# jonathan-laurent/AlphaZero.jl

Measured on AMD Instinct MI355X. Metric: self-play MCTS sims/sec (Connect-Four, 4096 parallel games per GPU), higher is better.
Workload: dtype f32

## Files before the change

### alphazero.jl_amd/csrc/azhip.hip

```cpp
#include "engine.h"
#include "minmax.h"

static thread_local std::string g_err;
int fail(int code, const char* fmt, ...) {
  char buf[512];
  va_list ap;
  va_start(ap, fmt);
  vsnprintf(buf, sizeof buf, fmt, ap);
  va_end(ap);
  g_err = buf;
  return code;
}
extern "C" const char* az_last_error(void) { return g_err.c_str(); }
extern "C" int az_debug_scratch_live_bytes(int64_t* bytes) {
  if (!bytes) return fail(AZ_ERR_BAD_ARG, "NULL argument");
  *bytes = (int64_t)scratch_live_bytes.load();
  return AZ_OK;
}
extern "C" int az_abi_version(void) { return AZ_ABI_VERSION; }
extern "C" int az_abi_struct_size(int32_t which) {
  switch (which) {
    case AZ_STRUCT_ENGINE_CFG: return (int)sizeof(az_engine_cfg);
    case AZ_STRUCT_MOVE_REC: return (int)sizeof(az_move_rec);
    case AZ_STRUCT_GAME_REC: return (int)sizeof(az_game_rec);
// ... 277 lines not shown
    long long plies = c->game == AZ_GAME_MANCALA ? 128 : gi.max_plies;
    cap = (long long)c->num_iters_per_turn * plies * std::max(1, c->reset_every);
    if (c->reset_every == 0) cap *= 4;
    cap = std::max<long long>(cap, 1024);
  }
  if (cap > (1LL << 30)) return fail(AZ_ERR_BAD_ARG, "max_nodes_per_slot too large");
  v.cap_nodes = (int)cap;
  int hs = 1024;
  while ((long long)hs * 2 < cap * 3) hs <<= 1;
  v.ht_size = hs;
  v.tag_mask = e->env.tag_mask; v.epoch0 = e->env.epoch0; v.bk_mode = e->env.bk_mode;
  AZCHK(dalloc(e, &v.sr, G)); AZCHK(dalloc(e, &v.game_id, G));
  AZCHK(dalloc(e, &v.move_idx, G)); AZCHK(dalloc(e, &e->d_node_count, G));
  AZCHK(dalloc(e, &v.worker_sim_id, G));
  AZCHK(dalloc(e, &v.eta, (size_t)G * gi.APAD));
  AZCHK(dalloc(e, &v.ht, (size_t)G * hs));
  AZCHK(create_node_pool(e));
  AZCHK(dalloc(e, &v.path, (size_t)G * v.max_depth));
  AZCHK(dalloc(e, &v.leaf_env, G));
  AZCHK(dalloc(e, &v.eval_slots, (size_t)2 * G)); v.eval_stride = G;
  AZCHK(dalloc(e, &v.bg_list, (size_t)2 * G)); AZCHK(dalloc(e, &v.bg_cnt, 2 * AZ_MAX_GROUPS));
  return dalloc(e, &v.n_eval, 2 * AZ_MAX_GROUPS);
}

static int create_side_records(az_engine* e) {
  DView& v = e->v; const int G = v.G;
  const size_t piece = (size_t)e->vm_chunk_nodes * 32;
  void* kbase = nullptr;
  bool mapped_keys = e->vm_rows > 0 && e->env.vmm_keys && piece > 0 && VM_CHUNK % piece == 0;
  size_t kbytes = 0;
  if (mapped_keys) {
    kbytes = ((size_t)e->vm_rows * G * piece + VM_CHUNK - 1) / VM_CHUNK * VM_CHUNK;
    if (hipMemAddressReserve(&kbase, kbytes, VM_CHUNK, nullptr, 0) != hipSuccess) { (void)hipGetLastError(); mapped_keys = false; }
  }
  if (mapped_keys) {
    e->vmk_base = (char*)kbase; e->vmk_bytes = kbytes; e->vmk_piece = piece;
    e->vmk_granule.assign(kbytes / VM_CHUNK, 0);
    v.keys = (unsigned long long*)kbase;
    v.key_row = (size_t)G * piece / 8; v.key_stride = piece / 8;
  } else {
    AZCHK(dalloc(e, &v.keys, (size_t)G * v.cap_nodes * 4, false));
    v.key_row = 0; v.key_stride = (size_t)v.cap_nodes * 4;
    if (e->vm_rows) v.key_row = (size_t)e->vm_chunk_nodes * 4;
  }
  hipLaunchKernelGGL(k_slot_records, dim3((G + 255) / 256), dim3(256), 0, e->stream, v, (int)SR_ZERO);
  return AZ_OK;
}

static int create_eval_cache(az_engine* e) {
  const az_engine_cfg* c = &e->cfg; const GameInfo& gi = e->gi; DView& v = e->v; const int G = v.G;
  AZCHK(dalloc(e, &v.Pout, (size_t)std::max(G, 1) * gi.APAD)); AZCHK(dalloc(e, &v.Vout, G));
  const bool on = e->env.eval_cache >= 0 ? e->env.eval_cache != 0 && c->oracle != AZ_ORACLE_ROLLOUT : oracle_is_net(*c);
  if (!on || e->env.use_graphs) return AZ_OK;
  int lg = e->env.eval_cache_log2;
  if (!lg) for (lg = 16; lg < 24 && ((long long)1 << lg) < 8LL * G * std::max(1, c->num_iters_per_turn);) ++lg;
  AZCHK(dalloc(e, &e->d_ec, (size_t)1 << lg));
  e->ec_mask = ((uint32_t)1 << lg) - 1u;
  AZCHK(dalloc(e, &e->d_ec_claim, (size_t)2 * G, false));
  HIPCHK(hipMemsetAsync(e->d_ec_claim, 0xff, sizeof(int) * 2 * (size_t)G, e->stream));
  AZCHK(dalloc(e, &e->d_Phit, (size_t)G * gi.APAD)); AZCHK(dalloc(e, &e->d_Vhit, G));
  v.ec = e->d_ec; v.ec_mask = e->ec_mask; v.ec_seq = 0; v.ec_claim = e->d_ec_claim; v.Phit = e->d_Phit; v.Vhit = e->d_Vhit;
  return AZ_OK;
}

static constexpr size_t FETCH_BYTES = (size_t)1 << 20;
static int create_words(az_engine* e) {
  DView& v = e->v; const int G = v.G;
  AZCHK(dalloc(e, &v.trace, (size_t)G * v.max_moves)); AZCHK(dalloc(e, &v.grec, G));
  AZCHK(dalloc(e, &v.finished, G)); AZCHK(dalloc(e, &v.err, 1));
  AZCHK(dalloc(e, &e->d_xerr, AZ_MAX_GROUPS + 1)); AZCHK(dalloc(e, &e->d_skipped, 2 * (AZ_MAX_GROUPS + 1)));
  v.xerr = e->d_xerr + AZ_MAX_GROUPS; v.skipped = e->d_skipped + 2 * AZ_MAX_GROUPS;
  AZCHK(halloc_mapped(e, &e->h_xflag, &e->d_xflag, 1, 0));
  AZCHK(halloc_mapped(e, &e->h_nleaf, &e->d_nleaf, AZ_MAX_GROUPS, -1));
  AZCHK(halloc_mapped(e, &e->h_needy, &e->d_needy, AZ_MAX_GROUPS, 0));
  AZCHK(dalloc(e, &e->d_fr, 1)); AZCHK(dalloc(e, &e->d_bg_stop, 1));
  AZCHK(halloc_mapped(e, &e->h_busy, &e->d_busy, AZ_MAX_GROUPS, -1));
  AZCHK(halloc_pinned(e, &e->h_report, 1, hipHostMallocMapped));
  memset(e->h_report, 0, sizeof *e->h_report);
  HIPCHK(hipHostGetDevicePointer((void**)&e->d_report, e->h_report, 0));
  AZCHK(halloc_pinned(e, &e->h_fetch, FETCH_BYTES));
  return halloc_mapped(e, &e->h_fr_words, &e->d_fr_words, 2, 0);
}

static int create_staging(az_engine* e) {
  const int G = e->v.G;
  e->io_cap = std::max(G, 4096);
  AZCHK(dalloc(e, &e->d_slots, e->io_cap)); AZCHK(dalloc(e, &e->d_gids, e->io_cap)); AZCHK(dalloc(e, &e->d_roots, e->io_cap));
  AZCHK(dalloc(e, &e->d_moves, e->io_cap)); AZCHK(dalloc(e, &e->d_eta, (size_t)e->io_cap * AZ_MAX_ACTIONS));
  AZCHK(dalloc(e, &e->d_offsets, e->io_cap)); AZCHK(dalloc(e, &e->d_stage, (size_t)G * e->v.max_moves));
  AZCHK(dalloc(e, &e->d_keys, (size_t)2 * e->io_cap)); AZCHK(dalloc(e, &e->d_actions, e->io_cap));
  AZCHK(dalloc(e, &e->d_next, (size_t)2 * e->io_cap)); AZCHK(dalloc(e, &e->d_term, e->io_cap)); AZCHK(dalloc(e, &e->d_reward, e->io_cap));
  AZCHK(dalloc(e, &e->d_nodebuf, 512));
  return dalloc(e, &e->d_visits, (size_t)e->io_cap * (AZ_MAX_ACTIONS + 1));
}

static int create_net_buffers(az_engine* e) {
  const az_engine_cfg* c = &e->cfg; const GameInfo& gi = e->gi;
  e->nn_cap = e->io_cap;
  if (c->oracle != AZ_ORACLE_SIMPLENET) AZCHK(dalloc(e, &e->d_hfeat, (size_t)e->nn_cap * gi.P * std::max(64, c->num_filters), false));
  AZCHK(dalloc(e, &e->d_X, (size_t)e->nn_cap * gi.C * gi.P)); AZCHK(dalloc(e, &e->d_A, (size_t)e->nn_cap * gi.A));
  AZCHK(dalloc(e, &e->d_P, (size_t)e->nn_cap * std::max(16, gi.APAD))); AZCHK(dalloc(e, &e->d_V, e->nn_cap)); AZCHK(dalloc(e, &e->d_Pinv, e->nn_cap));
  AZCHK(dalloc(e, &e->d_tmp_env, e->nn_cap)); AZCHK(dalloc(e, &e->d_iota, e->nn_cap)); AZCHK(dalloc(e, &e->d_ntmp, 1));
  AZCHK(halloc_pinned(e, &e->h_env, (size_t)e->nn_cap)); AZCHK(halloc_pinned(e, &e->h_n, 1)); AZCHK(halloc_pinned(e, &e->h_pv, (size_t)e->nn_cap * (gi.A + 1)));
  hipLaunchKernelGGL(k_iota, dim3((e->nn_cap + 255) / 256), dim3(256), 0, e->stream, e->d_iota, e->nn_cap);
  e->xch_epoch = e->env.xch_epoch0;
  { hipDeviceProp_t pr; HIPCHK(hipGetDeviceProperties(&pr, c->device)); e->num_cu = pr.multiProcessorCount; }
  return net_set_kernel_attrs(e);
}

static int create_groups(az_engine* e) {
  const az_engine_cfg* c = &e->cfg; const GameInfo& gi = e->gi; DView& v = e->v; const int G = v.G;
  if (e->env.tree_sort) { AZCHK(dalloc(e, &e->d_perm, (size_t)2 * G)); AZCHK(dalloc(e, &e->d_perm_prev, (size_t)2 * G)); }
  int ng = std::min(std::max(c->batch_size > 0 ? G / c->batch_size : 1, 1), (int)AZ_MAX_GROUPS);
  while (ng > 1 && G % ng != 0) --ng;
// ... 391 lines not shown
    HIPCHK(hipStreamSynchronize(e->stream));
  }
  HIPCHK(hipGetLastError());
  if (e->xch_epoch) AZCHK(check_device_error(e));
  return AZ_OK;
}

static int evaluate_envs(az_engine* e, const std::vector<GEnv>& envs, std::vector<float>& P, std::vector<float>& V) {
  const GameInfo& gi = e->gi;
  const int N = (int)envs.size();
  P.assign((size_t)N * gi.A, 0.f); V.assign(N, 0.f);
  for (int off = 0; off < N; off += e->nn_cap) {
    int m = std::min(e->nn_cap, N - off);
    HIPCHK(hipMemcpyAsync(e->d_tmp_env, envs.data() + off, sizeof(GEnv) * m, hipMemcpyHostToDevice, e->stream));
    HIPCHK(hipMemcpyAsync(e->d_ntmp, &m, sizeof(int), hipMemcpyHostToDevice, e->stream));
    AZCHK(seam_launch(e, false, m));
    HIPCHK(hipMemcpyAsync(P.data() + (size_t)gi.A * off, e->d_P, sizeof(float) * gi.A * m, hipMemcpyDeviceToHost, e->stream));
    HIPCHK(hipMemcpyAsync(V.data() + off, e->d_V, sizeof(float) * m, hipMemcpyDeviceToHost, e->stream));
    HIPCHK(hipStreamSynchronize(e->stream));
  }
  HIPCHK(hipGetLastError());
  if (e->xch_epoch) AZCHK(check_device_error(e));
  return AZ_OK;
}

extern "C" int az_net_evaluate_keys(az_engine* e, const uint64_t* keys, int32_t N, float* P, float* V) {
  ENGINE(e);
  if (!e->net_loaded) return fail(AZ_ERR_STATE, "az_net_set_params has not been called");
  if (N < 0 || (N > 0 && (!keys || !P || !V))) return fail(AZ_ERR_BAD_ARG, "NULL buffer");
  const GameInfo& gi = e->gi;
  for (int off = 0; off < N; off += e->nn_cap) {
    const int m = std::min(e->nn_cap, N - off);
    GEnv* envs = e->h_env;
    DISPATCH_GAME(e->cfg.game, { for (int i = 0; i < m; ++i) envs[i] = Gm::from_key(keys[2 * (size_t)(off + i)], keys[2 * (size_t)(off + i) + 1]); });
    *e->h_n = m;
    float* hP = e->h_pv; float* hV = e->h_pv + (size_t)gi.A * e->nn_cap;
    HIPCHK(hipMemcpyAsync(e->d_tmp_env, envs, sizeof(GEnv) * m, hipMemcpyHostToDevice, e->stream));
    HIPCHK(hipMemcpyAsync(e->d_ntmp, e->h_n, sizeof(int), hipMemcpyHostToDevice, e->stream));
    AZCHK(seam_launch(e, false, m));
    HIPCHK(hipMemcpyAsync(hP, e->d_P, sizeof(float) * gi.A * m, hipMemcpyDeviceToHost, e->stream));
    HIPCHK(hipMemcpyAsync(hV, e->d_V, sizeof(float) * m, hipMemcpyDeviceToHost, e->stream));
    HIPCHK(hipStreamSynchronize(e->stream));
    memcpy(P + (size_t)gi.A * off, hP, sizeof(float) * gi.A * m);
    memcpy(V + off, hV, sizeof(float) * m);
  }
  HIPCHK(hipGetLastError());
  if (e->xch_epoch) AZCHK(check_device_error(e));
  return AZ_OK;
}

static int ec_empty(az_engine* e, bool wipe) {
  if (!e->d_ec) return AZ_OK;
  AZCHK(sync_all(e));
  if (wipe) HIPCHK(hipMemsetAsync(e->d_ec, 0, sizeof(ECEnt) * ((size_t)e->ec_mask + 1), e->stream));
  HIPCHK(hipMemsetAsync(e->d_ec_claim, 0xff, sizeof(int) * 2 * (size_t)e->v.G, e->stream));
  HIPCHK(hipStreamSynchronize(e->stream));
  if (wipe) e->ec_seq = 0;
  e->v.ec_floor = e->ec_seq;
  for (int g = 0; g < e->ngroups; ++g) e->gv[g].ec_floor = e->ec_seq;
  return AZ_OK;
}
static int ec_next_launch(az_engine* e, DView* v) {
  if (!e->d_ec) return AZ_OK;
  if (e->ec_seq >= (1u << 29)) AZCHK(ec_empty(e, true));
  v->ec_seq = ++e->ec_seq;
  return AZ_OK;
}
template <class Gm> static int wave_group(az_engine* e, int g, uint32_t sim_idx) {
  constexpr int L = Gm::APAD;
  AZCHK(ec_next_launch(e, &e->gv[g]));
  const DView& v = e->gv[g];
  hipStream_t st = e->gs[g], sn = e->gt[g];
  const bool split = st != sn;
  const int G = v.G;
  const int gb = (G * L + 255) / 256;
  const int par = (e->wave_par[g] ^= 1);
  e->ph.stats.slot_launches += e->group_active[g];
  LAUNCH_ON(e, st, AZ_K_SELECT, G, (k_tree<Gm>), gb, 256, 0, v, e->p, (e->pending[g] || e->ph.fr_on) ? 1 : 0, 1, par);
  e->pending[g] = true;
  hipStream_t s2 = st;
  e->bg_signal = false;
  const bool side = e->ph.fr_on && !split && oracle_is_net(e->cfg) && e->fr_s[1] && st == e->fr_s[0];
  if (side) { s2 = e->fr_s[1]; HIPCHK(hipEventRecord(e->fr_ev[0], st)); ++e->bg_seq; e->bg_signal = env_process().bg_stop && e->ph.fr_kbg > 0; }
  if (oracle_is_net(e->cfg)) {
    AZCHK(net_wave(e, g, split, e->group_active[g]));
  } else {
    LAUNCH_ON(e, st, AZ_K_SYNTH, G, (k_synth_oracle<Gm>), (G + 255) / 256, 256, 0, v, e->p, sim_idx, par);
  }
  if (e->ph.fr_on) {
    FRArgs fa;
    fa.st = e->d_fr; fa.done = e->d_done; fa.done_off = e->d_done_off;
    fa.recs = e->d_phase ? e->d_phase : e->d_stage; fa.recs_cap = e->d_phase ? (long long)e->phase_cap : (long long)e->v.G * e->v.max_moves;
    fa.done_cap = e->done_cap; fa.total_games = e->ph.ids.total_games; fa.first_game_id = (uint32_t)e->ph.ids.first_game_id; fa.group = g; fa.host_words = e->d_fr_words;
    hipStream_t s3 = side ? e->fr_s[2] : s2;
    if (side) { HIPCHK(hipStreamWaitEvent(s2, e->fr_ev[0], 0)); HIPCHK(hipStreamWaitEvent(s3, e->fr_ev[0], 0)); }
    { DView mv = v; mv.low_prio = env_process().bg_prio ? 0 : 1; LAUNCH_ON(e, s3, AZ_K_MOVE, G, (k_move_fr<Gm>), (G + 255) / 256, 256, 0, mv, e->p, fa); }
    if (e->ph.fr_kbg > 0) {
      AZCHK(ec_next_launch(e, &e->gv[g]));
      DView bv = e->gv[g];
      bv.run_k = e->ph.fr_kbg; bv.low_prio = env_process().bg_prio ? 0 : 1;
      if (side && e->bg_signal) { bv.bg_stop = e->d_bg_stop; bv.bg_seq = e->bg_seq; }
      LAUNCH_ON(e, s2, AZ_K_EXPAND, G, (k_tree<Gm>), gb, 256, 0, bv, e->p, 0, 1, par ^ 1);
    }
    if (side) {
      HIPCHK(hipEventRecord(e->fr_ev[2], s3)); HIPCHK(hipStreamWaitEvent(s2, e->fr_ev[2], 0));
      HIPCHK(hipEventRecord(e->fr_ev[1], s2)); HIPCHK(hipStreamWaitEvent(st, e->fr_ev[1], 0));
    }
// ... 929 lines not shown
```

### alphazero.jl_amd/csrc/engine.h

```cpp
#pragma once
#include <hip/hip_runtime.h>

#include <algorithm>
#include <atomic>
#include <chrono>
#include <cmath>
#include <cstdarg>
#include <cstdio>
#include <cstring>
#include <new>
#include <string>
#include <map>
#include <memory>
#include <mutex>
#include <vector>
#include <unordered_set>

#include "../../include/az_numerics.h"
#include "../../include/azhip.h"
#include "env.h"
#include "games.h"
#include "net_layout.h"
#include "phase_books.h"
#include "resnet.h"
// ... 53 lines not shown
  return SimpleLayout(SimpleShape{gi.C * gi.P, gi.A, h.width, h.depth_common, h.depth_phead, h.depth_vhead, h.use_batch_norm});
}
inline bool oracle_is_net(const az_engine_cfg& c) { return c.oracle == AZ_ORACLE_RESNET || c.oracle == AZ_ORACLE_SIMPLENET; }

struct Phase {
  bool running = false;
  bool fr_on = false;
  bool host_moves = true;
  GameIds ids;
  int games_done = 0, wave_in_move = 0, active_slots = 0;
  int fr_k = 0, fr_kbg = 0, fr_round_waves = 0;
  int fr_prev_done = 0, fr_since_round = 0, fr_given_up = 0; long long fr_prev_recs = 0;
  int fr_look_waves = 0, fr_since_look = 0;
  std::vector<az_game_rec> q_games;
  std::vector<az_move_rec> q_moves;
  std::vector<az_game_rec> dev_games;
  std::vector<int64_t> dev_off; int64_t dev_n = 0;
  std::vector<int32_t> aborted_ids;
  az_selfplay_stats stats = {};
  std::chrono::steady_clock::time_point t_begin;
};
struct ProfRec { hipEvent_t a = nullptr, b = nullptr; int cls = 0; };
struct az_engine {
  az_engine_cfg cfg = {};
  az_simplenet_hp shp = {};
  GameInfo gi = {};
  EnvCreate env;
  int device = 0;
  hipStream_t stream = nullptr;
  DView v = {};
  DParams p = {};
  int ngroups = 0;
  DView gv[AZ_MAX_GROUPS] = {};
  hipStream_t gs[AZ_MAX_GROUPS] = {};
  hipStream_t gt[AZ_MAX_GROUPS] = {};
  hipEvent_t ev_tree[AZ_MAX_GROUPS] = {}, ev_net[AZ_MAX_GROUPS] = {};
  float* g_hfeat[AZ_MAX_GROUPS] = {};
  unsigned long long* xch[AZ_MAX_GROUPS + 1] = {}; unsigned long long xch_epoch = 0;
  int* d_xerr = nullptr; int* d_skipped = nullptr;
  int* h_needy = nullptr; int* d_needy = nullptr;
  int* h_nleaf = nullptr; int* d_nleaf = nullptr;
  int* h_xflag = nullptr; int* d_xflag = nullptr;
  bool split_off = false;
  long long xch_launches = 0;
  int split_registered = 0;
  std::vector<void*> allocs;
  size_t alloc_bytes = 0;
  std::vector<void*> host_allocs;
  char* vm_base = nullptr; size_t vm_bytes = 0, vm_chunk = 0; int vm_rows = 0, vm_chunk_nodes = 0;
  std::vector<hipMemGenericAllocationHandle_t> vm_handles; std::vector<char*> vm_at;
  std::vector<int> h_slot_cap, h_node_count; int* d_slot_cap = nullptr; int* d_node_count = nullptr; size_t vm_budget = 0, vm_mapped = 0;
  char* vmk_base = nullptr; size_t vmk_bytes = 0, vmk_piece = 0; std::vector<uint8_t> vmk_granule;
  int* d_perm = nullptr; long long* d_perm_prev = nullptr;
  ECEnt* d_ec = nullptr; uint32_t ec_mask = 0; uint32_t ec_seq = 0; int* d_ec_claim = nullptr; float* d_Phit = nullptr; float* d_Vhit = nullptr;
  size_t stat_words = 0; std::vector<long long> h_stat;
  std::vector<void*> net_allocs;
  bool net_loaded = false;
  std::vector<float> blob;
  std::unique_ptr<const NetMaps> net_maps;
  std::vector<unsigned char> trainable;
  NetDev net = {};
  std::unique_ptr<const SimpleMaps> simple_maps;
  SimpleDev snet = {};
  Net16bDev net16b = {};
  Net16Dev net16 = {};
  uint16_t* d_geo[GEO_COUNT] = {};
  long long tower_hist[4] = {};
  char last_tower[96] = {};
  int num_cu = 0;
  int nn_cap = 0;
  float* d_hfeat = nullptr; float* d_X = nullptr; float* d_A = nullptr; float* d_P = nullptr; float* d_V = nullptr; float* d_Pinv = nullptr;
  GEnv* d_tmp_env = nullptr; int* d_iota = nullptr; int* d_ntmp = nullptr;
  GEnv* h_env = nullptr; int* h_n = nullptr; float* h_pv = nullptr;
  int* d_slots = nullptr; uint32_t* d_gids = nullptr; GEnv* d_roots = nullptr; uint32_t* d_moves = nullptr; double* d_eta = nullptr; int* d_offsets = nullptr;
  az_move_rec* d_stage = nullptr; unsigned long long* d_keys = nullptr; int* d_actions = nullptr; unsigned long long* d_next = nullptr; signed char* d_term = nullptr; float* d_reward = nullptr;
  char* d_nodebuf = nullptr;
  int* d_visits = nullptr;
  int io_cap = 0;
  Phase ph;
  std::map<int, hipGraphExec_t> wave_graphs;
  bool pending[AZ_MAX_GROUPS] = {};
  int wave_par[AZ_MAX_GROUPS] = {};
  int group_active[AZ_MAX_GROUPS] = {};
  hipStream_t fr_s[4] = {}; hipEvent_t fr_ev[4] = {};
  FRState* d_fr = nullptr; az_game_rec* d_done = nullptr; long long* d_done_off = nullptr; int done_cap = 0;
  int* h_busy = nullptr; int* d_busy = nullptr;
  int* d_bg_stop = nullptr; int bg_seq = 0; bool bg_signal = false;
  int* h_fr_words = nullptr; int* d_fr_words = nullptr;
  std::vector<az_game_rec> h_done; std::vector<long long> h_done_off;
  StepReport* h_report = nullptr; StepReport* d_report = nullptr; bool report_fresh = false;
  char* h_fetch = nullptr;
  az_move_rec* d_phase = nullptr; int64_t phase_cap = 0;
  bool prof_on = false;
  int prof_mask = 0;
  std::vector<ProfRec> prof_pool;
  size_t prof_used = 0;
  az_prof prof = {};
  double next_exec = 1.0;
  std::vector<int> h_finished;
  std::vector<az_game_rec> h_grec;
  bool mm_on = false;
  az_minmax_cfg mm = {};
  GEnv* d_mm_roots = nullptr; double* d_mm_q = nullptr; int mm_cap = 0;
  unsigned long long* d_sv_keys = nullptr; int8_t* d_sv_q = nullptr; long long* d_sv_nodes = nullptr; int sv_cap = 0;
};

template <class T> inline int dalloc(az_engine* e, T** p, size_t n, bool zero = true) {
// ... 217 lines not shown
```

### alphazero.jl_amd/csrc/tree.h

```cpp
#pragma once
#include <hip/hip_runtime.h>
#include <stdint.h>
#include <type_traits>
#include "../../include/az_numerics.h"
#include "../../include/azhip.h"
#include "games.h"

enum { LEAF_NONE = 0, LEAF_NEW = 1, LEAF_TERMINAL = 2 };
enum { DERR_NODE_POOL = 1, DERR_HASH_FULL = 2, DERR_DEPTH = 3, DERR_MOVES = 4, DERR_NO_ROOT = 5 };

struct DParams {
  double gamma, cpuct, eps, alpha, prior_temp;
  int nsims, temp_len;
  int temp_xs[AZ_SCHED_MAX];
  double temp_ys[AZ_SCHED_MAX];
  uint64_t seed;
  int oracle, reset_every;
  double flip_p;
  int retire;
};

enum { SR_ACTIVE = 1, SR_MS_SHIFT = 8 };
struct alignas(64) SlotRec {
  unsigned long long root_a, root_b;
  long long tot_sims, tot_trav;
  uint32_t root_fin;
  int leaf_kd;
  int eidx, node_count;
  uint32_t epoch, leaf_ins;
  int root_idx, active;
  __host__ __device__ inline GEnv root() const { GEnv g; g.a = root_a; g.b = root_b; g.fin = root_fin; return g; }
  __host__ __device__ inline void set_root(const GEnv& g) { root_a = g.a; root_b = g.b; root_fin = g.fin; }
};
static_assert(sizeof(SlotRec) == 64, "slot record");

struct alignas(64) ECEnt { unsigned long long ka, kb; float P[AZ_MAX_ACTIONS]; float V; uint32_t cs; uint32_t meta; };
static_assert(sizeof(ECEnt) == 64, "evaluation cache entry");
enum { EC_EMPTY = 0, EC_PENDING = 1, EC_READY = 2, EC_FILLING = 3, EC_STALE_AFTER = 64 };

struct DView {
  int G, cap_nodes, ht_size, max_depth, max_moves;
  ECEnt* ec;
  uint32_t ec_mask, ec_seq;
  uint32_t ec_floor;
  int* ec_claim;
  int* needy_host;
  int* nleaf_host;
  float* Phit; float* Vhit;
  uint32_t tag_mask;
  uint32_t epoch0;
  SlotRec* sr;
  uint32_t* game_id;
  uint32_t* move_idx;
  int* worker_sim_id;
  double* eta;
  unsigned long long* ht;
  char* nodes;
  int node_sh; uint32_t node_mask; size_t node_row, node_stride;
  const int* slot_cap;
  unsigned long long* keys;
  size_t key_row, key_stride;
  const int* perm;
  int bk_mode;
  unsigned long long* path;
  GEnv* leaf_env;
  int* eval_slots;
  int eval_stride;
  const int* bg_stop; int bg_seq;
  int* bg_list; int* bg_cnt;
  int* n_eval;
  float* Pout;
  float* Vout;
  az_move_rec* trace;
  az_game_rec* grec;
  int* finished;
  int* err;
  int* xerr;
  int* skipped;
  long long* stat;
  unsigned long long* dbg;
  int run_k;
  int fr;
  int* busy_host;
  int low_prio;
  int slot0;
  int* fr_active;
};

static constexpr int AZ_MAX_GROUPS = 4;
struct FRState {
  unsigned long long resv;
  long long moves;
  int next_game;
  int active[AZ_MAX_GROUPS];
};
struct FRArgs {
// ... 45 lines not shown
  static_assert(L == 8 || L == 16, "lane groups of 8 or 16");
  x += dpp_partner<0>(x);
  x += dpp_partner<1>(x);
  x += dpp_partner<2>(x);
  if constexpr (L == 16) x += dpp_partner<3>(x);
  return x;
}
template <int CTRL> __device__ __forceinline__ double dpp_ctrl(double x) {
  const int lo = __builtin_amdgcn_update_dpp(0, __double2loint(x), CTRL, 0xF, 0xF, false);
  const int hi = __builtin_amdgcn_update_dpp(0, __double2hiint(x), CTRL, 0xF, 0xF, false);
  return __hiloint2double(hi, lo);
}
template <int L> __device__ __forceinline__ int group_argmax(double s, int lane, int* carry) {
  static_assert(L == 8 || L == 16, "lane groups of 8 or 16");
  constexpr int Q1 = 0xB1, Q2 = 0x4E, HM = 0x141, RM = 0x140;
  double m = __builtin_fmax(s, dpp_ctrl<Q1>(s));
  m = __builtin_fmax(m, dpp_ctrl<Q2>(m));
  m = __builtin_fmax(m, dpp_ctrl<HM>(m));
  if constexpr (L == 16) m = __builtin_fmax(m, dpp_ctrl<RM>(m));
  const unsigned long long eq = __ballot(s == m);
  const int base = (threadIdx.x & 63) & ~(L - 1);
  const int idx = __ffs((unsigned)((eq >> base) & ((1u << L) - 1u))) - 1;
  int c = (lane == idx) ? *carry : 0;
  c |= __builtin_amdgcn_update_dpp(0, c, Q1, 0xF, 0xF, false);
  c |= __builtin_amdgcn_update_dpp(0, c, Q2, 0xF, 0xF, false);
  c |= __builtin_amdgcn_update_dpp(0, c, HM, 0xF, 0xF, false);
  if constexpr (L == 16) c |= __builtin_amdgcn_update_dpp(0, c, RM, 0xF, 0xF, false);
  *carry = c;
  return idx;
}
template <int L> __device__ __forceinline__ int group_argmax(double s, int lane) { int c = 0; return group_argmax<L>(s, lane, &c); }

template <int L> __device__ __forceinline__ uint32_t group_xor(uint32_t x) {
  x ^= (uint32_t)dpp_partner<0>((int)x);
  x ^= (uint32_t)dpp_partner<1>((int)x);
  x ^= (uint32_t)dpp_partner<2>((int)x);
  if constexpr (L == 16) x ^= (uint32_t)dpp_partner<3>((int)x);
  return x;
}
template <int L> __device__ __forceinline__ int group_bcast0(int x, int lane) { return group_sum<L>(lane == 0 ? x : 0); }
__device__ __forceinline__ uint32_t ec_ld32(const uint32_t* p) { return __hip_atomic_load(p, __ATOMIC_RELAXED, __HIP_MEMORY_SCOPE_AGENT); }
__device__ __forceinline__ unsigned long long ec_ld64(const unsigned long long* p) { return __hip_atomic_load(p, __ATOMIC_RELAXED, __HIP_MEMORY_SCOPE_AGENT); }
__device__ __forceinline__ float ec_ldf(const float* p) { return __uint_as_float(__hip_atomic_load((const uint32_t*)p, __ATOMIC_RELAXED, __HIP_MEMORY_SCOPE_AGENT)); }
__device__ __forceinline__ void ec_st32(uint32_t* p, uint32_t v) { __hip_atomic_store(p, v, __ATOMIC_RELAXED, __HIP_MEMORY_SCOPE_AGENT); }
__device__ __forceinline__ void ec_st64(unsigned long long* p, unsigned long long v) { __hip_atomic_store(p, v, __ATOMIC_RELAXED, __HIP_MEMORY_SCOPE_AGENT); }
__device__ __forceinline__ void ec_stf(float* p, float v) { __hip_atomic_store((uint32_t*)p, __float_as_uint(v), __ATOMIC_RELAXED, __HIP_MEMORY_SCOPE_AGENT); }
__device__ __forceinline__ bool ec_cas(uint32_t* p, uint32_t expect, uint32_t want) {
  return __hip_atomic_compare_exchange_strong(p, &expect, want, __ATOMIC_RELAXED, __ATOMIC_RELAXED, __HIP_MEMORY_SCOPE_AGENT);
}
__device__ __forceinline__ uint32_t ec_term(float p, int lane) {
  const uint32_t b = __float_as_uint(p), r = (uint32_t)(5 * lane + 1) & 31u;
  return (b << r) | (b >> ((32u - r) & 31u));
}
__device__ __forceinline__ uint32_t ec_checksum(uint32_t px, unsigned long long ka, unsigned long long kb, float V, uint32_t ready_meta) {
  unsigned long long h = az_hash_key(ka, kb);
  h = az_mix64(h ^ (((unsigned long long)px << 32) | (unsigned long long)__float_as_uint(V)));
  h = az_mix64(h + (unsigned long long)ready_meta);
  return (uint32_t)(h >> 32) ^ (uint32_t)h;
}
__device__ __forceinline__ uint32_t ec_index(unsigned long long ka, unsigned long long kb, uint32_t mask) {
  return (uint32_t)(az_hash_key(ka, kb) >> 17) & mask;
}

template <class Gm>
__device__ inline int ht_lookup(const DView& v, int slot, int lane, unsigned long long ka,
                                unsigned long long kb, uint32_t epoch, uint32_t* ins) {
  constexpr int L = Gm::APAD;
  const unsigned long long hk = az_hash_key(ka, kb);
  const uint32_t H1 = (uint32_t)v.ht_size - 1;
  const uint32_t h0 = (uint32_t)hk & H1;
  const uint32_t tag = (uint32_t)(hk >> 40) & v.tag_mask;
  const unsigned long long* tab = v.ht + (size_t)slot * v.ht_size;
  const int iters = v.ht_size / L;
  for (int i = 0; i < iters; ++i) {
    uint32_t pos = (h0 + (uint32_t)(i * L + lane)) & H1;
    unsigned long long e = tab[pos];
    uint32_t idx1 = (uint32_t)e;
    bool live = ((uint32_t)(e >> 48) == epoch) && idx1 != 0;
    bool match = false;
    if (live && ((uint32_t)(e >> 32) & 0xffff) == tag) {
      const unsigned long long* k = side_at(v, slot, (int)(idx1 - 1));
      match = (k[0] == ka) && (k[1] == kb);
    }
    unsigned mb = group_ballot<L>(match), db = group_ballot<L>(!live);
    int fm = mb ? __ffs(mb) - 1 : 99, fd = db ? __ffs(db) - 1 : 99;
    if (fm < fd) {
      int base = (threadIdx.x & 63) & ~(L - 1);
      return (int)__shfl((int)idx1, base + fm) - 1;
    }
    if (fd != 99) { *ins = (h0 + (uint32_t)(i * L + fd)) & H1; return -1; }
  }
  dev_fail(v, DERR_HASH_FULL);
  *ins = 0;
  return -1;
}

template <class Gm>
__device__ inline void arm_noise(const DView& v, const DParams& p, int slot, const GEnv& env) {
  constexpr int L = Gm::APAD;
  uint32_t m = Gm::mask(env);
  int n = __popc(m);
  double eta[AZ_MAX_ACTIONS];
  az_rng r = az_rng_make(p.seed, v.game_id[slot], v.move_idx[slot], AZ_RNG_NOISE);
  az_dirichlet(&r, n, p.alpha, eta);
  int k = 0;
  for (int a = 0; a < L; ++a) {
    double e = 0.0;
    if (a < Gm::A && ((m >> a) & 1)) e = eta[k++];
    v.eta[(size_t)slot * L + a] = e;
  }
}

template <class Gm> __device__ inline void set_link(char* nd, int act, uint32_t link) {
  using NL = NodeL<Gm>;
  ((uint16_t*)(nd + NL::OFF_LO))[act] = (uint16_t)(link & 0xffff);
// ... 29 lines not shown
  unsigned long long st = (v.path + (size_t)slot_in * v.max_depth)[lane < v.max_depth ? lane : 0];
  GEnv lenv = v.leaf_env[slot_in];
  int kind = s0.leaf_kd & 3, depth = (s0.leaf_kd >> 2) & 0x0fffffff, e0 = s0.eidx, nc = s0.node_count;
  GEnv root0 = s0.root();
  uint32_t epoch0 = s0.epoch, ins = s0.leaf_ins;
  int ridx = s0.root_idx, active0 = s0.active;
  int claim0 = -1; uint32_t cmeta0 = 0;
  if (v.ec) { const int2 c2 = ((const int2*)v.ec_claim)[slot_in]; claim0 = c2.x; cmeta0 = (uint32_t)c2.y; }
#define AZ_PIN(x) asm volatile("" : "+v"(x))
  AZ_PIN(kind); AZ_PIN(depth); AZ_PIN(e0); AZ_PIN(nc); AZ_PIN(st); AZ_PIN(root0.a); AZ_PIN(root0.b); AZ_PIN(root0.fin);
  AZ_PIN(epoch0); AZ_PIN(ins); AZ_PIN(claim0); AZ_PIN(cmeta0); AZ_PIN(lenv.a); AZ_PIN(lenv.b); AZ_PIN(lenv.fin); AZ_PIN(ridx); AZ_PIN(active0);
  const bool mine = live && !(v.fr && kind != LEAF_NONE && (!do_backup || ((s0.leaf_kd >> 30) & 1) == par));
  if (!(do_backup && mine)) kind = LEAF_NONE;
  const int nc_in = nc, ridx_in = ridx;
  const bool inrec = lane < Gm::A;
  float Pans = 0.f, Vans = 0.f;
  if (kind == LEAF_NEW) {
    Pans = e0 >= 0 ? v.Pout[(size_t)e0 * L + lane] : v.Phit[(size_t)slot_in * L + lane];
    Vans = e0 >= 0 ? v.Vout[e0] : v.Vhit[slot_in];
  }
  const bool searching = mine && (active0 & SR_ACTIVE);
  int msims = active0 >> SR_MS_SHIFT;
  int done_sims = 0, done_trav = 0;
  int n_sel = 0, n_trav = 0, n_evl = 0, n_hit = 0;
  bool retired = false, ishit = false;
  int claim = -1; uint32_t cmeta = 0;

  for (int it = 0;; ++it) {
    KArgs ka;
    {
      auto kp = __builtin_amdgcn_kernarg_segment_ptr();
      asm volatile("" : "+s"(kp));
      __builtin_memcpy(&ka, (const void*)kp, sizeof(KArgs));
    }
    const DView& v = ka.v;
    const DParams& p = ka.p;
    int slot = slot_in; asm volatile("" : "+v"(slot));
    unsigned long long* const path = v.path + (size_t)slot * v.max_depth;
    if (kind != LEAF_NONE) {
      double q = 0.0;
      bool ok = true;
      if (kind == LEAF_NEW) {
        const int idx = nc;
        if (it == 0 && v.ec && claim0 >= 0) {
          ECEnt* const ent = v.ec + claim0;
          const float Praw = inrec ? Pans : 0.f;
          const uint32_t fill = (cmeta0 & ~3u) | EC_FILLING, ready = (cmeta0 & ~3u) | EC_READY;
          int got = 0;
          if (lane == 0) got = ec_cas(&ent->meta, cmeta0, fill) ? 1 : 0;
          got = group_bcast0<L>(got, lane);
          const uint32_t px = group_xor<L>(inrec ? ec_term(Praw, lane) : 0u);
          if (got) {
            if (inrec) ec_stf(&ent->P[lane], Praw);
            if (lane == 0) { ec_stf(&ent->V, Vans); ec_st32(&ent->cs, ec_checksum(px, lenv.a, lenv.b, Vans, ready)); }
            __builtin_amdgcn_s_waitcnt(0);
            if (lane == 0) ec_st32(&ent->meta, ready);
          }
        }
        if (idx >= (v.slot_cap ? v.slot_cap[slot] : v.cap_nodes)) {
          ok = false;
          if (!p.retire) dev_fail(v, DERR_NODE_POOL);
          else {
            retired = true;
            if (lane == 0) { v.finished[slot] = 2; if (v.fr_active) atomicSub(v.fr_active, 1); }
          }
        } else {
          const uint32_t m = Gm::mask(lenv);
          float Pf = Pans;
          if (p.prior_temp != 1.0) {
            const bool av = (m >> lane) & 1;
            double res;
            if (p.prior_temp == 0.0) {
              int am = group_argmax<L>(av ? (double)Pf : -__builtin_inf(), lane);
              res = (lane == am) ? 1.0 : 0.0;
            } else {
              double pw = av ? az_pow((double)Pf, 1.0 / p.prior_temp) : 0.0;
              double sm = 0.0;
              for (int a = 0; a < Gm::A; ++a) { double t = __shfl(pw, gbase + a); if ((m >> a) & 1) sm += t; }
              res = pw / sm;
            }
            Pf = av ? (float)res : 0.f;
          }
          if (depth == 0) ridx = idx;
          char* nd = node_at<Gm>(v, slot, idx);
          const unsigned long long st_par = (depth >= 1 && depth <= L) ? __shfl(st, gbase + depth - 1) : (depth > L ? path[depth - 1] : 0ULL);
          if (lane < Gm::A) {
            *NL::stat(nd, lane) = typename NL::Stat{0.0, 0, Pf};
            ((uint16_t*)(nd + NL::OFF_LO))[lane] = 0;
          }
          if (lane == 0) {
            *(typename NL::hi_t*)(nd + NL::OFF_HI) = 0;
            unsigned long long* kk = side_at(v, slot, idx);
            kk[0] = lenv.a; kk[1] = lenv.b; kk[2] = (unsigned long long)__float_as_uint(Vans);
            const unsigned long long hk = az_hash_key(lenv.a, lenv.b);
            const unsigned long long tag = (hk >> 40) & v.tag_mask;
            v.ht[(size_t)slot * v.ht_size + ins] =
                ((unsigned long long)epoch0 << 48) | (tag << 32) | (unsigned long long)(idx + 1);
            if (depth != 0 && links_ok)
              set_link<Gm>(node_at<Gm>(v, slot, (int)(uint32_t)st_par), (int)((st_par >> 32) & 0xff), (uint32_t)(idx + 1));
          }
          nc = idx + 1;
          q = (double)Vans;
        }
      }
      if (ok) {
        for (int c = (depth - 1) / L; c >= 0 && depth > 0; --c) {
          const int k0 = c * L, kn = (depth - k0) < L ? (depth - k0) : L;
// ... 52 lines not shown
          else if (lane == 0 && links_ok) set_link<Gm>(node_at<Gm>(v, slot, pidx), pact, (uint32_t)(idx + 1));
          have = false;
        }
        if (depth >= v.max_depth) { dev_fail(v, DERR_DEPTH); kind = LEAF_NONE; break; }
        if (!have) {
          const char* nd = node_at<Gm>(v, slot, idx);
          if (inrec) { sa = *NL::stat(nd, lane); lo = ((const uint16_t*)(nd + NL::OFF_LO))[lane]; }
          hi = *(const typename NL::hi_t*)(nd + NL::OFF_HI);
        }
        const uint32_t amask = Gm::mask(env);
        const int N = sa.N;
        const float Pf = sa.P;
        const double W = sa.W;
        const int link = (int)(lo | (((hi >> (2 * lane)) & 3u) << 16));
        if (dbg && it == 0 && depth == 0) dbg[2] = __builtin_readcyclecounter() + (unsigned long long)(N & 0);
        const int Ntot = group_sum<L>(N);
        const double sqrtNtot = __builtin_sqrt((double)Ntot);
        const double Q = W / (double)(N > 1 ? N : 1);
        double Pd = (double)Pf;
        if (depth == 0 && p.eps != 0.0) Pd = (1.0 - p.eps) * Pd + p.eps * v.eta[(size_t)slot * L + lane];
        double sc = Q + p.cpuct * Pd * sqrtNtot / (double)(N + 1);
        if (!((amask >> lane) & 1)) sc = -__builtin_inf();
        int nxt = link;
        if (dbg && it == 0 && depth == 0) dbg[7] = __builtin_readcyclecounter() + (unsigned long long)(__double2loint(sc) & 0);
        const int act = group_argmax<L>(sc, lane, &nxt);
        if (dbg && it == 0 && depth == 0) dbg[8] = __builtin_readcyclecounter() + (unsigned long long)(act & 0);
        have = nxt != 0;
        if (have) {
          const char* nd = node_at<Gm>(v, slot, nxt - 1);
          if (inrec) { sa = *NL::stat(nd, lane); lo = ((const uint16_t*)(nd + NL::OFF_LO))[lane]; }
          hi = *(const typename NL::hi_t*)(nd + NL::OFF_HI);
        }
        const bool wp = Gm::white_playing(env);
        Gm::play(env, act);
        const float wr = Gm::white_reward(env);
        const int r = (int)(wp ? wr : -wr);
        const bool psw = wp != Gm::white_playing(env);
        const unsigned long long ent = (unsigned long long)(uint32_t)idx | ((unsigned long long)act << 32) |
                                       ((unsigned long long)(psw ? 1 : 0) << 40) | ((unsigned long long)(r + 1) << 41);
        if (lane == 0) path[depth] = ent;
        if (lane == depth) st = ent;
        pidx = idx; pact = act;
        if (dbg && it == 0 && depth == 0) dbg[9] = __builtin_readcyclecounter() + (env.a & 0);
        depth++;
        probe = nxt == 0;
        idx = nxt - 1;
      }
      if (dbg && it == 0) dbg[3] = __builtin_readcyclecounter();
      lenv = env;
      if (kind != LEAF_NONE) { n_sel += 1; n_trav += depth; }
      if (kind == LEAF_NEW) {
        n_evl += 1;
        if (v.ec) {
          const uint32_t ci = ec_index(env.a, env.b, v.ec_mask);
          ECEnt* const ent = v.ec + ci;
          const uint32_t m1 = ec_ld32(&ent->meta);
          const unsigned long long ka = ec_ld64(&ent->ka), kb = ec_ld64(&ent->kb);
          const float pl = inrec ? ec_ldf(&ent->P[lane]) : 0.f;
          const float vv = ec_ldf(&ent->V);
          const uint32_t cs = ec_ld32(&ent->cs);
          const uint32_t px = group_xor<L>(inrec ? ec_term(pl, lane) : 0u);
          const bool okc = (m1 & 3u) == EC_READY && (m1 >> 2) > v.ec_floor && ka == env.a && kb == env.b && cs == ec_checksum(px, ka, kb, vv, m1);
          ishit = group_bcast0<L>(okc ? 1 : 0, lane) != 0;
          if (ishit) { Pans = inrec ? pl : 0.f; Vans = vv; n_hit += 1; }
          else {
            claim = -1; cmeta = 0;
            if (lane == 0) {
              const int32_t age = (int32_t)(v.ec_seq - (m1 >> 2));
              if (m1 == 0u || (m1 & 3u) == EC_READY || age > (int32_t)EC_STALE_AFTER || (m1 >> 2) <= v.ec_floor) {
                const uint32_t mine = (v.ec_seq << 2) | EC_PENDING;
                if (ec_cas(&ent->meta, m1, mine)) { ec_st64(&ent->ka, env.a); ec_st64(&ent->kb, env.b); claim = (int)ci; cmeta = mine; }
              }
            }
          }
        }
      }
    }
    if (kind == LEAF_NONE) break;
    if (kind == LEAF_NEW && !ishit) break;
    if (!v.run_k) break;
    __threadfence_block();
  }

  const int slot = slot_in;
  SlotRec* const sr = v.sr + slot;
  if (mine && lane == 0) {
    sr->leaf_kd = kind == LEAF_NONE ? (int)LEAF_NONE : (kind | (depth << 2) | (par << 30));
    if (do_select && kind != LEAF_NONE) { v.leaf_env[slot] = lenv; sr->leaf_ins = ins; }
    if (nc != nc_in) sr->node_count = nc;
    if (ridx != ridx_in) sr->root_idx = ridx;
    if (done_sims) { sr->tot_trav += done_trav; sr->tot_sims += done_sims; }
    const int aw = retired ? 0 : ((active0 & ((1 << SR_MS_SHIFT) - 1)) | (msims << SR_MS_SHIFT));
    if (aw != active0) sr->active = aw;
  }
  if (!do_select) return;
  if (ishit && kind == LEAF_NEW) {
    v.Phit[(size_t)slot * L + lane] = Pans;
    if (lane == 0) { v.Vhit[slot] = Vans; sr->eidx = -1; }
  }
  if (dbg) dbg[4] = __builtin_readcyclecounter();

  const bool head = mine && lane == 0;
  const bool isnew = head && kind == LEAF_NEW && !ishit;
  const unsigned long long bal = __ballot(isnew);
  const bool needy = head && v.run_k && v.bg_list && (v.fr ? (do_backup && searching && !retired && kind == LEAF_NONE && msims < p_arg.nsims)
                                                           : (kind != LEAF_NONE || (searching && !retired && msims < p_arg.nsims)));
  const unsigned long long baln = __ballot(needy);
  int sims = head ? n_sel : 0, trav = head ? n_trav : 0, evl = head ? n_evl : 0, hits = head ? n_hit : 0;
#pragma unroll
  for (int o = 32; o > 0; o >>= 1) { sims += __shfl_down(sims, o); trav += __shfl_down(trav, o); evl += __shfl_down(evl, o); hits += __shfl_down(hits, o); }
  if (wl == 0) { s_need[w] = __popcll(baln); s_new[w] = __popcll(bal); s_hit[w] = hits; s_evl[w] = evl; s_sims[w] = sims; s_trav[w] = trav; }
  __syncthreads();
  if (threadIdx.x == 0) {
    const int nw = blockDim.x >> 6;
    int tot = 0, toth = 0, te = 0, ts = 0, tt = 0;
    for (int i = 0; i < nw; ++i) { tot += s_new[i]; toth += s_hit[i]; te += s_evl[i]; ts += s_sims[i]; tt += s_trav[i]; }
    s_base = tot ? atomicAdd(v.n_eval + par, tot) : 0;
    { int tn = 0; for (int i = 0; i < nw; ++i) tn += s_need[i]; s_nbase = tn ? atomicAdd(v.bg_cnt + par, tn) : 0; }
    if (ts) {
      long long* sp = v.stat + (size_t)blockIdx.x * 4;
      sp[0] += ts; sp[1] += tt; sp[2] += te; sp[3] += toth;
    }
    if (blockIdx.x == 0 && (do_backup || !v.fr)) {
      if (v.nleaf_host && do_select) __hip_atomic_store(v.nleaf_host, v.n_eval[par ^ 1], __ATOMIC_RELAXED, __HIP_MEMORY_SCOPE_SYSTEM);
// ... 430 lines not shown
```

Measured before the change: 8.974 million.

## Make eval cache two-way set-associative and size it from free device memory

Turns the direct-mapped evaluation cache into a 2-way set-associative cache. A lookup probes both ways of a set, and a victim-selection rule prefers free, then stale, then older answered entries, and avoids evicting fresh pending claims. The default table size can now grow past 2^24 toward 2^27 entries, up to 64x the number of simulations, capped at one eighth of free device memory. The goal is a higher hit rate so fewer leaves need network evaluation, at the cost of an extra entry load per probe, more memory, and a larger wipe.

```diff
diff --git a/alphazero.jl_amd/csrc/azhip.hip b/alphazero.jl_amd/csrc/azhip.hip
--- a/alphazero.jl_amd/csrc/azhip.hip
+++ b/alphazero.jl_amd/csrc/azhip.hip
@@ -353,14 +353,15 @@
   AZCHK(dalloc(e, &v.Pout, (size_t)std::max(G, 1) * gi.APAD)); AZCHK(dalloc(e, &v.Vout, G));
   const bool on = e->env.eval_cache >= 0 ? e->env.eval_cache != 0 && c->oracle != AZ_ORACLE_ROLLOUT : oracle_is_net(*c);
   if (!on || e->env.use_graphs) return AZ_OK;
-  int lg = e->env.eval_cache_log2;
-  if (!lg) for (lg = 16; lg < 24 && ((long long)1 << lg) < 8LL * G * std::max(1, c->num_iters_per_turn);) ++lg;
-  AZCHK(dalloc(e, &e->d_ec, (size_t)1 << lg));
-  e->ec_mask = ((uint32_t)1 << lg) - 1u;
+  size_t free_b = 0, total_b = 0;
+  HIPCHK(hipMemGetInfo(&free_b, &total_b));
+  const int lg = ec_size_log2(G, c->num_iters_per_turn, e->env.eval_cache_log2, (unsigned long long)free_b);
+  e->ec_entries = (size_t)1 << lg;
+  AZCHK(dalloc(e, &e->d_ec, e->ec_entries));
   AZCHK(dalloc(e, &e->d_ec_claim, (size_t)2 * G, false));
   HIPCHK(hipMemsetAsync(e->d_ec_claim, 0xff, sizeof(int) * 2 * (size_t)G, e->stream));
   AZCHK(dalloc(e, &e->d_Phit, (size_t)G * gi.APAD)); AZCHK(dalloc(e, &e->d_Vhit, G));
-  v.ec = e->d_ec; v.ec_mask = e->ec_mask; v.ec_seq = 0; v.ec_claim = e->d_ec_claim; v.Phit = e->d_Phit; v.Vhit = e->d_Vhit;
+  v.ec = e->d_ec; v.ec_set_mask = (uint32_t)(e->ec_entries / EC_WAYS) - 1u; v.ec_seq = 0; v.ec_claim = e->d_ec_claim; v.Phit = e->d_Phit; v.Vhit = e->d_Vhit;
   return AZ_OK;
 }
 
@@ -858,7 +859,7 @@
 static int ec_empty(az_engine* e, bool wipe) {
   if (!e->d_ec) return AZ_OK;
   AZCHK(sync_all(e));
-  if (wipe) HIPCHK(hipMemsetAsync(e->d_ec, 0, sizeof(ECEnt) * ((size_t)e->ec_mask + 1), e->stream));
+  if (wipe) HIPCHK(hipMemsetAsync(e->d_ec, 0, sizeof(ECEnt) * e->ec_entries, e->stream));
   HIPCHK(hipMemsetAsync(e->d_ec_claim, 0xff, sizeof(int) * 2 * (size_t)e->v.G, e->stream));
   HIPCHK(hipStreamSynchronize(e->stream));
   if (wipe) e->ec_seq = 0;
diff --git a/alphazero.jl_amd/csrc/engine.h b/alphazero.jl_amd/csrc/engine.h
--- a/alphazero.jl_amd/csrc/engine.h
+++ b/alphazero.jl_amd/csrc/engine.h
@@ -129,7 +129,7 @@
   std::vector<int> h_slot_cap, h_node_count; int* d_slot_cap = nullptr; int* d_node_count = nullptr; size_t vm_budget = 0, vm_mapped = 0;
   char* vmk_base = nullptr; size_t vmk_bytes = 0, vmk_piece = 0; std::vector<uint8_t> vmk_granule;
   int* d_perm = nullptr; long long* d_perm_prev = nullptr;
-  ECEnt* d_ec = nullptr; uint32_t ec_mask = 0; uint32_t ec_seq = 0; int* d_ec_claim = nullptr; float* d_Phit = nullptr; float* d_Vhit = nullptr;
+  ECEnt* d_ec = nullptr; size_t ec_entries = 0; uint32_t ec_seq = 0; int* d_ec_claim = nullptr; float* d_Phit = nullptr; float* d_Vhit = nullptr;
   size_t stat_words = 0; std::vector<long long> h_stat;
   std::vector<void*> net_allocs;
   bool net_loaded = false;
diff --git a/alphazero.jl_amd/csrc/eval_cache_rule.h b/alphazero.jl_amd/csrc/eval_cache_rule.h
--- /dev/null
+++ b/alphazero.jl_amd/csrc/eval_cache_rule.h
@@ -0,0 +1,53 @@
+#pragma once
+#include <cstdint>
+
+#include "../../include/az_numerics.h"
+
+#ifdef __HIPCC__
+#define EC_HD __host__ __device__ inline
+#else
+#define EC_HD inline
+#endif
+
+enum { EC_EMPTY = 0, EC_PENDING = 1, EC_READY = 2, EC_FILLING = 3, EC_STALE_AFTER = 64 };
+enum { EC_ENTRY_BYTES = 64, EC_WAYS = 2, EC_LINE_BYTES = EC_ENTRY_BYTES * EC_WAYS };
+
+EC_HD uint32_t ec_set_of_hash(uint64_t hk, uint32_t set_mask) { return (uint32_t)(hk >> 17) & set_mask; }
+EC_HD uint32_t ec_set_of(uint64_t ka, uint64_t kb, uint32_t set_mask) { return ec_set_of_hash(az_hash_key(ka, kb), set_mask); }
+
+EC_HD uint32_t ec_checksum(uint32_t px, uint64_t hk, float V, uint32_t ready_meta) {
+  uint64_t h = az_mix64(hk ^ (((uint64_t)px << 32) | (uint64_t)az_f2u(V)));
+  h = az_mix64(h + (uint64_t)ready_meta);
+  return (uint32_t)(h >> 32) ^ (uint32_t)h;
+}
+
+EC_HD bool ec_way_hit(uint32_t meta, uint32_t floor, uint64_t ka, uint64_t kb, float V, uint32_t cs, uint32_t px,
+                      uint64_t key_a, uint64_t key_b, uint64_t hk) {
+  return (meta & 3u) == EC_READY && (meta >> 2) > floor && ka == key_a && kb == key_b && cs == ec_checksum(px, hk, V, meta);
+}
+
+enum { EC_WAY_FREE = 0, EC_WAY_STALE = 1, EC_WAY_ANSWERED = 2, EC_WAY_FRESH = 3 };
+EC_HD int ec_way_class(uint32_t meta, uint32_t seq, uint32_t floor) {
+  const uint32_t n = meta >> 2;
+  return meta == 0u || n <= floor ? EC_WAY_FREE : (meta & 3u) == EC_READY ? EC_WAY_ANSWERED
+       : (int32_t)(seq - n) > (int32_t)EC_STALE_AFTER ? EC_WAY_STALE : EC_WAY_FRESH;
+}
+EC_HD int ec_pick_victim(uint32_t meta0, uint32_t meta1, bool same0, bool same1, uint32_t seq, uint32_t floor) {
+  const int c0 = ec_way_class(meta0, seq, floor), c1 = ec_way_class(meta1, seq, floor);
+  const bool barred = (c0 == EC_WAY_FRESH && (same0 || c1 == EC_WAY_FRESH)) || (c1 == EC_WAY_FRESH && same1);
+  const bool second_is_older = (int32_t)(seq - (meta1 >> 2)) > (int32_t)(seq - (meta0 >> 2));
+  const int w = c0 != c1 ? (c0 < c1 ? 0 : 1) : (c0 == EC_WAY_ANSWERED && second_is_older) ? 1 : 0;
+  return barred ? -1 : w;
+}
+
+enum { EC_MIN_LOG2 = 16, EC_SMALL_CAP_LOG2 = 24, EC_BIG_MULT = 64, EC_BIG_CAP_LOG2 = 27 };
+inline int ec_size_log2(int G, int sims, int override_log2, unsigned long long free_bytes) {
+  if (override_log2 > 0) return override_log2 < 4 ? 4 : override_log2 > 28 ? 28 : override_log2;
+  const long long work = (long long)(G > 0 ? G : 1) * (sims > 0 ? sims : 1);
+  int lg = EC_MIN_LOG2;
+  while (lg < EC_SMALL_CAP_LOG2 && (1LL << lg) < 8LL * work) ++lg;
+  if (lg == EC_SMALL_CAP_LOG2)
+    while (lg < EC_BIG_CAP_LOG2 && (1LL << lg) < (long long)EC_BIG_MULT * work) ++lg;
+  while (lg > EC_MIN_LOG2 && ((unsigned long long)EC_ENTRY_BYTES << lg) > free_bytes / 8) --lg;
+  return lg;
+}
diff --git a/alphazero.jl_amd/csrc/tree.h b/alphazero.jl_amd/csrc/tree.h
--- a/alphazero.jl_amd/csrc/tree.h
+++ b/alphazero.jl_amd/csrc/tree.h
@@ -3,6 +3,7 @@
 #include <stdint.h>
 #include <type_traits>
 #include "../../include/az_numerics.h"
+#include "eval_cache_rule.h"
 #include "../../include/azhip.h"
 #include "games.h"
 
@@ -36,12 +37,12 @@
 
 struct alignas(64) ECEnt { unsigned long long ka, kb; float P[AZ_MAX_ACTIONS]; float V; uint32_t cs; uint32_t meta; };
 static_assert(sizeof(ECEnt) == 64, "evaluation cache entry");
-enum { EC_EMPTY = 0, EC_PENDING = 1, EC_READY = 2, EC_FILLING = 3, EC_STALE_AFTER = 64 };
+static_assert(sizeof(ECEnt) == EC_ENTRY_BYTES, "eval_cache_rule.h sizes the table in entries of this size");
 
 struct DView {
   int G, cap_nodes, ht_size, max_depth, max_moves;
   ECEnt* ec;
-  uint32_t ec_mask, ec_seq;
+  uint32_t ec_set_mask, ec_seq;
   uint32_t ec_floor;
   int* ec_claim;
   int* needy_host;
@@ -193,15 +194,6 @@
   const uint32_t b = __float_as_uint(p), r = (uint32_t)(5 * lane + 1) & 31u;
   return (b << r) | (b >> ((32u - r) & 31u));
 }
-__device__ __forceinline__ uint32_t ec_checksum(uint32_t px, unsigned long long ka, unsigned long long kb, float V, uint32_t ready_meta) {
-  unsigned long long h = az_hash_key(ka, kb);
-  h = az_mix64(h ^ (((unsigned long long)px << 32) | (unsigned long long)__float_as_uint(V)));
-  h = az_mix64(h + (unsigned long long)ready_meta);
-  return (uint32_t)(h >> 32) ^ (uint32_t)h;
-}
-__device__ __forceinline__ uint32_t ec_index(unsigned long long ka, unsigned long long kb, uint32_t mask) {
-  return (uint32_t)(az_hash_key(ka, kb) >> 17) & mask;
-}
 
 template <class Gm>
 __device__ inline int ht_lookup(const DView& v, int slot, int lane, unsigned long long ka,
@@ -337,7 +329,7 @@
           const uint32_t px = group_xor<L>(inrec ? ec_term(Praw, lane) : 0u);
           if (got) {
             if (inrec) ec_stf(&ent->P[lane], Praw);
-            if (lane == 0) { ec_stf(&ent->V, Vans); ec_st32(&ent->cs, ec_checksum(px, lenv.a, lenv.b, Vans, ready)); }
+            if (lane == 0) { ec_stf(&ent->V, Vans); ec_st32(&ent->cs, ec_checksum(px, az_hash_key(lenv.a, lenv.b), Vans, ready)); }
             __builtin_amdgcn_s_waitcnt(0);
             if (lane == 0) ec_st32(&ent->meta, ready);
           }
@@ -496,24 +488,29 @@
       if (kind == LEAF_NEW) {
         n_evl += 1;
         if (v.ec) {
-          const uint32_t ci = ec_index(env.a, env.b, v.ec_mask);
-          ECEnt* const ent = v.ec + ci;
-          const uint32_t m1 = ec_ld32(&ent->meta);
-          const unsigned long long ka = ec_ld64(&ent->ka), kb = ec_ld64(&ent->kb);
-          const float pl = inrec ? ec_ldf(&ent->P[lane]) : 0.f;
-          const float vv = ec_ldf(&ent->V);
-          const uint32_t cs = ec_ld32(&ent->cs);
-          const uint32_t px = group_xor<L>(inrec ? ec_term(pl, lane) : 0u);
-          const bool okc = (m1 & 3u) == EC_READY && (m1 >> 2) > v.ec_floor && ka == env.a && kb == env.b && cs == ec_checksum(px, ka, kb, vv, m1);
-          ishit = group_bcast0<L>(okc ? 1 : 0, lane) != 0;
-          if (ishit) { Pans = inrec ? pl : 0.f; Vans = vv; n_hit += 1; }
+          const unsigned long long hk = az_hash_key(env.a, env.b);
+          const uint32_t ci = 2u * ec_set_of_hash(hk, v.ec_set_mask);
+          ECEnt* const e0 = v.ec + ci;
+          ECEnt* const e1 = e0 + 1;
+          const uint32_t m0 = ec_ld32(&e0->meta), m1 = ec_ld32(&e1->meta);
+          const unsigned long long ka0 = ec_ld64(&e0->ka), kb0 = ec_ld64(&e0->kb), ka1 = ec_ld64(&e1->ka), kb1 = ec_ld64(&e1->kb);
+          const float pl0 = inrec ? ec_ldf(&e0->P[lane]) : 0.f, pl1 = inrec ? ec_ldf(&e1->P[lane]) : 0.f;
+          const float vv0 = ec_ldf(&e0->V), vv1 = ec_ldf(&e1->V);
+          const uint32_t cs0 = ec_ld32(&e0->cs), cs1 = ec_ld32(&e1->cs);
+          const uint32_t px0 = group_xor<L>(inrec ? ec_term(pl0, lane) : 0u), px1 = group_xor<L>(inrec ? ec_term(pl1, lane) : 0u);
+          const int okw = ec_way_hit(m0, v.ec_floor, ka0, kb0, vv0, cs0, px0, env.a, env.b, hk) ? 1
+                        : ec_way_hit(m1, v.ec_floor, ka1, kb1, vv1, cs1, px1, env.a, env.b, hk) ? 2 : 0;
+          const int hitw = group_bcast0<L>(okw, lane);
+          ishit = hitw != 0;
+          if (ishit) { Pans = hitw == 1 ? pl0 : pl1; Vans = hitw == 1 ? vv0 : vv1; n_hit += 1; }
           else {
             claim = -1; cmeta = 0;
             if (lane == 0) {
-              const int32_t age = (int32_t)(v.ec_seq - (m1 >> 2));
-              if (m1 == 0u || (m1 & 3u) == EC_READY || age > (int32_t)EC_STALE_AFTER || (m1 >> 2) <= v.ec_floor) {
+              const int w = ec_pick_victim(m0, m1, ka0 == env.a && kb0 == env.b, ka1 == env.a && kb1 == env.b, v.ec_seq, v.ec_floor);
+              if (w >= 0) {
+                ECEnt* const ent = w ? e1 : e0;
                 const uint32_t mine = (v.ec_seq << 2) | EC_PENDING;
-                if (ec_cas(&ent->meta, m1, mine)) { ec_st64(&ent->ka, env.a); ec_st64(&ent->kb, env.b); claim = (int)ci; cmeta = mine; }
+                if (ec_cas(&ent->meta, w ? m1 : m0, mine)) { ec_st64(&ent->ka, env.a); ec_st64(&ent->kb, env.b); claim = (int)ci + w; cmeta = mine; }
               }
             }
           }
```

Result: faster. 10.61 million, median of 6 (+18.2%).
